# sndels/prosper

Measured on AMD Instinct MI355X. Metric: Mpaths/s, higher is better.
Workload: dtype f32; 1 GPU; S-cornell 1920x1080 8spp maxBounces 4; width=1920, height=1080, spp=8, max_bounces=4, triangles=38, bvh_nodes=7, parallelism=image stripes x1, pipeline=wavefront, 3 frames in flight (one launch chain each)

## Files before the change

include/prosper_pt/prosper_pt.h:

```cpp
#ifndef PROSPER_PT_H
#define PROSPER_PT_H

#include <stddef.h>
#include <stdint.h>

#include "shader_structs.h"

#ifdef __cplusplus
extern "C" {
#endif

#define PROSPER_PT_ABI_VERSION 4

enum
{
    PROSPER_PT_OK = 0,
    PROSPER_PT_ERR_INVALID_ARGUMENT = -1,
    PROSPER_PT_ERR_NO_DEVICE = -2,
    PROSPER_PT_ERR_HIP = -3,
    PROSPER_PT_ERR_NO_SCENE = -4,
    PROSPER_PT_ERR_SCENE = -5,
    PROSPER_PT_ERR_UNSUPPORTED = -6,
    PROSPER_PT_NOT_READY = -7,
};
// ... 969 lines not shown
int prosper_pt_comm_init(prosper_pt_ctx *ctx, const uint8_t id[PROSPER_PT_COMM_ID_BYTES], uint32_t rank, uint32_t ranks);
int prosper_pt_comm_adopt(prosper_pt_ctx *ctx, void *nccl_comm, uint32_t rank, uint32_t ranks);
int prosper_pt_comm_destroy(prosper_pt_ctx *ctx);
int prosper_pt_gather_tiles(
    prosper_pt_ctx *ctx, uint32_t root, void *device_full_rgba32f, size_t byte_size, uint32_t flags, void *stream);
int prosper_pt_gather_wait(prosper_pt_ctx *ctx, void *stream);
typedef struct prosper_pt_comm_info
{
    uint32_t ranks;
    uint32_t rank;
    int32_t device;
    uint32_t gathers;
    float lastGatherMs;
    uint32_t reserved;
} prosper_pt_comm_info;
int prosper_pt_comm_query(prosper_pt_ctx *ctx, prosper_pt_comm_info *out);
int prosper_pt_get_gathered_device_ptr(prosper_pt_ctx *ctx, void **out_ptr, uint32_t *width, uint32_t *height);
int prosper_pt_read_gathered(prosper_pt_ctx *ctx, float *rgba32f, size_t byte_size, void *stream);
int prosper_pt_deinterleave_tiles(
    prosper_pt_ctx *ctx, const void *device_tiles, uint32_t ranks, uint32_t stripe_width, uint32_t width, uint32_t height,
    void *device_full_rgba32f, size_t byte_size, void *stream);

int prosper_pt_get_counters(prosper_pt_ctx *ctx, prosper_pt_counters *out, void *stream);
int prosper_pt_get_stage_counters(prosper_pt_ctx *ctx, uint32_t stage, prosper_pt_counters *out, void *stream);
int prosper_pt_reset_counters(prosper_pt_ctx *ctx, void *stream);

#define PROSPER_PT_MAX_KERNELS 8
int prosper_pt_get_last_render_ms(prosper_pt_ctx *ctx, float *total_ms, float kernel_ms[PROSPER_PT_MAX_KERNELS]);
int prosper_pt_get_last_render_timing(
    prosper_pt_ctx *ctx, float *total_ms, float kernel_ms[PROSPER_PT_MAX_KERNELS],
    uint32_t kernel_launches[PROSPER_PT_MAX_KERNELS]);
const char *prosper_pt_kernel_name(uint32_t index);
int prosper_pt_set_kernel_timing(prosper_pt_ctx *ctx, int enabled);

enum
{
    PROSPER_PT_FN_SINCOS = 0,
    PROSPER_PT_FN_POW = 1,
    PROSPER_PT_FN_SRGB_TO_LINEAR = 2,
    PROSPER_PT_FN_NORMALIZE = 3,
    PROSPER_PT_FN_UNPACK_SNORM = 4,
    PROSPER_PT_FN_ONB = 5,
    PROSPER_PT_FN_COSINE_SAMPLE = 6,
    PROSPER_PT_FN_VNDF_SAMPLE = 7,
    PROSPER_PT_FN_VNDF_PDF = 8,
    PROSPER_PT_FN_EVAL_BRDF = 9,
    PROSPER_PT_FN_OFFSET_RAY = 10,
    PROSPER_PT_FN_POINT_LIGHT = 11,
    PROSPER_PT_FN_SPOT_LIGHT = 12,
    PROSPER_PT_FN_TRIANGLE = 13,
    PROSPER_PT_FN_HALF = 14,
    PROSPER_PT_FN_RNG = 15,
    PROSPER_PT_FN_BC7_BLOCK = 16,
    PROSPER_PT_FN_COUNT = 17,
};

int prosper_pt_debug_srgb_monotonicity(
    prosper_pt_ctx *ctx, uint32_t first_bits, uint32_t last_bits, float *max_defect, uint64_t *decreases);

int prosper_pt_eval_device_fn(
    prosper_pt_ctx *ctx, uint32_t fn, const float *in, uint32_t in_stride, float *out,
    uint32_t out_stride, uint32_t n);

#ifdef __cplusplus
}
#endif

#endif
```

prosper_amd/csrc/prosper_pt.cpp:

```cpp
#include "../../include/prosper_pt/prosper_pt.h"

#include <hip/hip_runtime.h>

#include <algorithm>
#include <chrono>
#include <future>
#include <memory>
#include <cmath>
#include <cstdlib>
#include <cstdio>
#include <cstring>
#include <exception>
#include <stdexcept>
#include <string>
#include <vector>

#include "bvh_build.hpp"
#include "pt_animation.hpp"
#include "pt_context.hpp"
#include "pt_geometry.hpp"
#include "pt_kernels.hpp"
#include "pt_materials.hpp"
#include "pt_pass_support.hpp"
#include "pt_scene.hpp"
// ... 1539 lines not shown
    float total = 0.0f;
    if (const int rc = ctx->timeline.add_to(perStage, launches, &total)) return rc;
    if (perStage[kStageChains] > 0.0f || launches[kStageChains] > 0)
    {
        uint32_t chainLaunches = 0;
        float chainMs = 0.0f;
        for (const LaunchTimeline &chain : ctx->slots[ctx->timedSlot].chains)
        {
            if (const int rc = chain.add_to(perStage, launches, &chainMs)) return rc;
            chainLaunches += chain.intervals();
        }
        if (chainLaunches)
        {
            perStage[kStageChains] = 0.0f;
            launches[kStageChains] = 0;
        }
    }
    *total_ms = total;
    for (int i = 0; i < PROSPER_PT_MAX_KERNELS; ++i)
    {
        if (kernel_ms) kernel_ms[i] = perStage[i];
        if (kernel_launches) kernel_launches[i] = launches[i];
    }
    return PROSPER_PT_OK;
}

int prosper_pt_debug_srgb_monotonicity(
    prosper_pt_ctx *ctx, uint32_t first_bits, uint32_t last_bits, float *max_defect, uint64_t *decreases)
{
    if (!ctx || !max_defect || !decreases || first_bits > last_bits || last_bits >= 0x7F800000u)
        return fail(PROSPER_PT_ERR_INVALID_ARGUMENT, "prosper_pt_debug_srgb_monotonicity: bad argument");
    PPT_HIP(hipSetDevice(ctx->device));
    uint32_t *d = nullptr;
    PPT_HIP(hipMalloc((void **)&d, 8));
    hipError_t e = hipMemset(d, 0, 8);
    uint32_t host[2] = {0u, 0u};
    if (e == hipSuccess)
    {
        launch_srgb_monotonicity(first_bits, last_bits, d, nullptr);
        e = hipGetLastError();
    }
    if (e == hipSuccess) e = hipMemcpy(host, d, 8, hipMemcpyDeviceToHost);
    (void)hipFree(d);
    PPT_HIP(e);
    std::memcpy(max_defect, &host[0], 4);
    *decreases = host[1];
    return PROSPER_PT_OK;
}

int prosper_pt_eval_device_fn(
    prosper_pt_ctx *ctx, uint32_t fn, const float *in, uint32_t in_stride, float *out, uint32_t out_stride, uint32_t n)
{
    if (!ctx || !in || !out || fn >= PROSPER_PT_FN_COUNT || in_stride == 0 || out_stride == 0 ||
        (fn == PROSPER_PT_FN_BC7_BLOCK && (in_stride < 4 || out_stride < 16)))
        return fail(PROSPER_PT_ERR_INVALID_ARGUMENT, "prosper_pt_eval_device_fn: bad argument");
    PPT_HIP(hipSetDevice(ctx->device));
    float *dIn = nullptr, *dOut = nullptr;
    const size_t inBytes = (size_t)n * in_stride * 4, outBytes = (size_t)n * out_stride * 4;
    PPT_HIP(hipMalloc((void **)&dIn, inBytes + 16));
    hipError_t e = hipMalloc((void **)&dOut, outBytes + 16);
    if (e == hipSuccess) e = hipMemcpy(dIn, in, inBytes, hipMemcpyHostToDevice);
    if (e == hipSuccess) e = hipMemset(dOut, 0, outBytes + 16);
    if (e == hipSuccess)
    {
        launch_eval_fn(fn, dIn, in_stride, dOut, out_stride, n, nullptr);
        e = hipGetLastError();
    }
    if (e == hipSuccess) e = hipMemcpy(out, dOut, outBytes, hipMemcpyDeviceToHost);
    (void)hipFree(dIn);
    (void)hipFree(dOut);
    if (e != hipSuccess) return fail(PROSPER_PT_ERR_HIP, std::string("eval_device_fn: ") + hipGetErrorString(e));
    return PROSPER_PT_OK;
}

}
```

prosper_amd/csrc/pt_device.hpp:

```cpp
#pragma once

#include "pt_math.hpp"
#include "pt_scene.hpp"

namespace ppt
{

#define PPT_D __device__ __forceinline__

constexpr uint32_t kMissIndex = 0xFFFFFFFFu;

struct LaneCounters
{
    uint32_t closestRays, shadowRays, nodeVisits, triangleTests, closestHits, anyHitCalls, lightSamples,
        spotLightSamples, skyLookups, shortIndexHits, paths, pixelsWritten, historyReads, shortIndexTriangleTests,
        nodePhaseSteps, trianglePhaseSteps, anyHitTexelFetches;
};


PPT_D uint32_t pcg(uint32_t v)
{
    const uint32_t state = v * 747796405u + 2891336453u;
    const uint32_t word = ((state >> ((state >> 28) + 4u)) ^ state) * 277803737u;
    return (word >> 22) ^ word;
// ... 1452 lines not shown
{
    const float tMaxK = tMax * kSlabTol;
    e[0] = slab_entry(tnx01.x, tny01.x, tnz01.x, tfx01.x, tfy01.x, tfz01.x, tMin, tMaxK);
    e[1] = slab_entry(tnx01.y, tny01.y, tnz01.y, tfx01.y, tfy01.y, tfz01.y, tMin, tMaxK);
    e[2] = slab_entry(tnx23.x, tny23.x, tnz23.x, tfx23.x, tfy23.x, tfz23.x, tMin, tMaxK);
    e[3] = slab_entry(tnx23.y, tny23.y, tnz23.y, tfx23.y, tfy23.y, tfz23.y, tMin, tMaxK);
    ref[0] = (int32_t)children.x;
    ref[1] = (int32_t)children.y;
    ref[2] = (int32_t)children.z;
    ref[3] = (int32_t)children.w;
#define PPT_CSWAP(i, j)                                                                                                \
    {                                                                                                                  \
        const bool sw = e[j] < e[i];                                                                                   \
        const float te = sw ? e[j] : e[i];                                                                             \
        e[j] = sw ? e[i] : e[j];                                                                                       \
        e[i] = te;                                                                                                     \
        const int32_t tr = sw ? ref[j] : ref[i];                                                                       \
        ref[j] = sw ? ref[i] : ref[j];                                                                                 \
        ref[i] = tr;                                                                                                   \
    }
    if constexpr (SORTED)
    {
        PPT_CSWAP(0, 1)
        PPT_CSWAP(2, 3)
        PPT_CSWAP(0, 2)
        PPT_CSWAP(1, 3)
        PPT_CSWAP(1, 2)
    }
#undef PPT_CSWAP
}

template <bool SORTED = true>
PPT_D void intersect_node4(const NodeData &n, f3 o, const RaySlabs &rs, float tMin, float tMax, float e[4], int32_t ref[4])
{
    const float ox = o.x - __builtin_bit_cast(float, n.q0.x);
    const float oy = o.y - __builtin_bit_cast(float, n.q0.y);
    const float oz = o.z - __builtin_bit_cast(float, n.q0.z);
    const bool sx = rs.invd.x < 0.0f, sy = rs.invd.y < 0.0f, sz = rs.invd.z < 0.0f;
    const uint32_t nx01 = sx ? n.q2.z : n.q1.x, nx23 = sx ? n.q2.w : n.q1.y;
    const uint32_t fx01 = sx ? n.q1.x : n.q2.z, fx23 = sx ? n.q1.y : n.q2.w;
    const uint32_t ny01 = sy ? n.q3.x : n.q1.z, ny23 = sy ? n.q3.y : n.q1.w;
    const uint32_t fy01 = sy ? n.q1.z : n.q3.x, fy23 = sy ? n.q1.w : n.q3.y;
    const uint32_t nz01 = sz ? n.q3.z : n.q2.x, nz23 = sz ? n.q3.w : n.q2.y;
    const uint32_t fz01 = sz ? n.q2.x : n.q3.z, fz23 = sz ? n.q2.y : n.q3.w;
    const v2f tnx01 = plane_offsets(nx01, ox) * rs.invd.x, tnx23 = plane_offsets(nx23, ox) * rs.invd.x;
    const v2f tny01 = plane_offsets(ny01, oy) * rs.invd.y, tny23 = plane_offsets(ny23, oy) * rs.invd.y;
    const v2f tnz01 = plane_offsets(nz01, oz) * rs.invd.z, tnz23 = plane_offsets(nz23, oz) * rs.invd.z;
    const v2f tfx01 = plane_offsets(fx01, ox) * rs.invdK.x, tfx23 = plane_offsets(fx23, ox) * rs.invdK.x;
    const v2f tfy01 = plane_offsets(fy01, oy) * rs.invdK.y, tfy23 = plane_offsets(fy23, oy) * rs.invdK.y;
    const v2f tfz01 = plane_offsets(fz01, oz) * rs.invdK.z, tfz23 = plane_offsets(fz23, oz) * rs.invdK.z;
    finish_node4<SORTED>(tnx01, tnx23, tny01, tny23, tnz01, tnz23, tfx01, tfx23, tfy01, tfy23, tfz01, tfz23, n.q4, tMin, tMax, e, ref);
}

struct GlobalGeom
{
    const BvhNode *nodes;
    const WorldTriangle *triangles;
    PPT_D NodeData node(int32_t i) const
    {
        const uint4 *np = reinterpret_cast<const uint4 *>(nodes + i);
        return NodeData{np[0], np[1], np[2], np[3], np[4]};
    }
    template <bool SORTED>
    PPT_D void test_node(int32_t i, f3 o, const RaySlabs &rs, float tMin, float tMax, float e[4], int32_t ref[4]) const
    {
        intersect_node4<SORTED>(node(i), o, rs, tMin, tMax, e, ref);
    }
    PPT_D TriangleData tri(uint32_t i) const
    {
        const float4 *tp = reinterpret_cast<const float4 *>(triangles + i);
        return TriangleData{tp[0], tp[1], tp[2]};
    }
};
constexpr uint32_t kLdsNodeStride = 9;
struct LdsGeom
{
    const float4 *nodes;
    const float4 *triangles;
    template <bool SORTED>
    PPT_D void test_node(int32_t i, f3 o, const RaySlabs &rs, float tMin, float tMax, float e[4], int32_t ref[4]) const
    {
        typedef float f4n __attribute__((ext_vector_type(4)));
        typedef uint32_t u4n __attribute__((ext_vector_type(4)));
        typedef __attribute__((address_space(3))) const f4n *lds_f4;
        typedef __attribute__((address_space(3))) const u4n *lds_u4;
        const uint32_t base = (uint32_t)(uintptr_t)(__attribute__((address_space(3))) const void *)nodes + (uint32_t)i * (kLdsNodeStride * 16u);
        const uint32_t sx = (__builtin_bit_cast(uint32_t, rs.invd.x) >> 25) & 64u;
        const uint32_t sy = (__builtin_bit_cast(uint32_t, rs.invd.y) >> 25) & 64u;
        const uint32_t sz = (__builtin_bit_cast(uint32_t, rs.invd.z) >> 25) & 64u;
        const f4n origin = *(lds_f4)(uintptr_t)(base);
        const f4n nx = *(lds_f4)(uintptr_t)(base + 16u + sx), fx = *(lds_f4)(uintptr_t)(base + 80u - sx);
        const f4n ny = *(lds_f4)(uintptr_t)(base + 32u + sy), fy = *(lds_f4)(uintptr_t)(base + 96u - sy);
        const f4n nz = *(lds_f4)(uintptr_t)(base + 48u + sz), fz = *(lds_f4)(uintptr_t)(base + 112u - sz);
        const u4n ch = *(lds_u4)(uintptr_t)(base + 64u);
        const uint4 children = make_uint4(ch.x, ch.y, ch.z, ch.w);
        const float ox = o.x - origin.x, oy = o.y - origin.y, oz = o.z - origin.z;
        const v2f tnx01 = v2f{nx.x - ox, nx.y - ox} * rs.invd.x, tnx23 = v2f{nx.z - ox, nx.w - ox} * rs.invd.x;
        const v2f tny01 = v2f{ny.x - oy, ny.y - oy} * rs.invd.y, tny23 = v2f{ny.z - oy, ny.w - oy} * rs.invd.y;
        const v2f tnz01 = v2f{nz.x - oz, nz.y - oz} * rs.invd.z, tnz23 = v2f{nz.z - oz, nz.w - oz} * rs.invd.z;
        const v2f tfx01 = v2f{fx.x - ox, fx.y - ox} * rs.invdK.x, tfx23 = v2f{fx.z - ox, fx.w - ox} * rs.invdK.x;
        const v2f tfy01 = v2f{fy.x - oy, fy.y - oy} * rs.invdK.y, tfy23 = v2f{fy.z - oy, fy.w - oy} * rs.invdK.y;
        const v2f tfz01 = v2f{fz.x - oz, fz.y - oz} * rs.invdK.z, tfz23 = v2f{fz.z - oz, fz.w - oz} * rs.invdK.z;
        finish_node4<SORTED>(tnx01, tnx23, tny01, tny23, tnz01, tnz23, tfx01, tfx23, tfy01, tfy23, tfz01, tfz23, children, tMin, tMax, e, ref);
    }
    PPT_D TriangleData tri(uint32_t i) const
    {
        const float4 *tp = triangles + i * 3u;
        return TriangleData{tp[0], tp[1], tp[2]};
    }
};
constexpr uint32_t kLdsNodeStrideHalf = 5;
struct LdsGeomHalf
{
    const float4 *nodes;
    const float4 *triangles;
    PPT_D NodeData node(int32_t i) const
    {
        const uint4 *np = reinterpret_cast<const uint4 *>(nodes + (uint32_t)i * kLdsNodeStrideHalf);
        return NodeData{np[0], np[1], np[2], np[3], np[4]};
    }
    template <bool SORTED>
    PPT_D void test_node(int32_t i, f3 o, const RaySlabs &rs, float tMin, float tMax, float e[4], int32_t ref[4]) const
    {
        intersect_node4<SORTED>(node(i), o, rs, tMin, tMax, e, ref);
    }
    PPT_D TriangleData tri(uint32_t i) const
    {
        const float4 *tp = triangles + i * 3u;
        return TriangleData{tp[0], tp[1], tp[2]};
    }
};
constexpr uint32_t kLdsSceneFloat4s = 768;

PPT_D bool descend_any(const float e[4], const int32_t ref[4], const TraversalStack &stack, int32_t &sp, int32_t &node)
{
    bool found = false;
    if (stack.ldsOnly || (uint32_t)sp + 3u <= stack.cap)
    {
#pragma unroll
        for (int k = 0; k < 4; ++k)
            if (e[k] < kInf)
            {
                if (found)
                    stack.lds[(uint32_t)(sp++) * stack.ldsStride] = ref[k];
                else
                {
                    node = ref[k];
                    found = true;
                }
            }
        return found;
    }
#pragma unroll
    for (int k = 0; k < 4; ++k)
        if (e[k] < kInf)
        {
            if (found)
                stack.push(sp, ref[k]);
            else
            {
                node = ref[k];
                found = true;
            }
        }
    return found;
}

enum BlendPolicy : uint32_t
{
    kBlendStochastic = 0,
    kBlendReject = 1,
    kBlendPeel = 2,
};
PPT_D bool ascending(f3 a, f3 b)
{
    return a.x < b.x || (a.x == b.x && (a.y < b.y || (a.y == b.y && a.z < b.z)));
}

template <bool ANY, bool COUNT, class Geom, BlendPolicy BLEND = kBlendStochastic>
PPT_D bool trace_in(
    const Geom &g, const DeviceScene &s, f3 o, f3 d, float tMin, float tMaxIn, uint32_t seed, const TraversalStack &stack,
    Hit &hit, LaneCounters &cnt, const Hit *after = nullptr)
// ... 309 lines not shown
```

prosper_amd/csrc/pt_kernels.hip:

```cpp
#include "pt_kernels.hpp"

#include "bvh_encode.hpp"
#include "pt_bc7.hpp"
#include "pt_device.hpp"
#include "pt_render_common.hpp"

namespace ppt
{


__global__ void flatten_triangles_kernel(
    DeviceScene s, const uint32_t *__restrict__ triOffsets, uint32_t drawInstanceCount,
    const uint32_t *__restrict__ drawInstanceFlags, WorldTriangle *__restrict__ out,
    ShadeTriangle *__restrict__ shadeOut, AlphaTriangle *__restrict__ alphaOut, uint32_t total,
    const uint32_t *__restrict__ leafPosition, WorldTriangle *__restrict__ leafOrder)
{
    const uint32_t g = blockIdx.x * blockDim.x + threadIdx.x;
    if (g >= total) return;
    uint32_t lo = 0, hi = drawInstanceCount;
    while (hi - lo > 1)
    {
        const uint32_t mid = (lo + hi) >> 1;
        if (triOffsets[mid] <= g)
            lo = mid;
// ... 557 lines not shown
        break;
    case PROSPER_PT_FN_EVAL_BRDF:
    {
        Surface sf = {};
        sf.normalWS = f3{a[3], a[4], a[5]};
        sf.invViewRayWS = f3{a[6], a[7], a[8]};
        sf.material.albedo = f3{a[9], a[10], a[11]};
        sf.material.roughness = a[12];
        sf.material.metallic = a[13];
        sf.NoV = saturate(dot(sf.normalWS, sf.invViewRayWS));
        const f3 r = eval_brdf_times_nol(f3{a[0], a[1], a[2]}, sf);
        o[0] = r.x; o[1] = r.y; o[2] = r.z;
        break;
    }
    case PROSPER_PT_FN_OFFSET_RAY:
    {
        const f3 r = offset_ray(f3{a[0], a[1], a[2]}, f3{a[3], a[4], a[5]});
        o[0] = r.x; o[1] = r.y; o[2] = r.z;
        break;
    }
    case PROSPER_PT_FN_POINT_LIGHT:
    {
        prosper_PointLight L;
        L.position = prosper_vec4{a[0], a[1], a[2], 0.0f};
        L.radianceAndRadius = prosper_vec4{a[3], a[4], a[5], a[6]};
        f3 l, irr;
        float d;
        eval_point_light(L, f3{a[7], a[8], a[9]}, l, d, irr);
        o[0] = l.x; o[1] = l.y; o[2] = l.z; o[3] = d; o[4] = irr.x; o[5] = irr.y; o[6] = irr.z;
        break;
    }
    case PROSPER_PT_FN_SPOT_LIGHT:
    {
        prosper_SpotLight L;
        L.positionAndAngleOffset = prosper_vec4{a[0], a[1], a[2], a[3]};
        L.radianceAndAngleScale = prosper_vec4{a[4], a[5], a[6], a[7]};
        L.direction = prosper_vec4{a[8], a[9], a[10], 0.0f};
        f3 l, irr;
        float d;
        eval_spot_light(L, f3{a[11], a[12], a[13]}, l, d, irr);
        o[0] = l.x; o[1] = l.y; o[2] = l.z; o[3] = d; o[4] = irr.x; o[5] = irr.y; o[6] = irr.z;
        break;
    }
    case PROSPER_PT_FN_TRIANGLE:
    {
        float t = 0.0f, bu = 0.0f, bv = 0.0f;
        const f3 dir = f3{a[3], a[4], a[5]};
        const bool hit = intersect_triangle(
            f3{a[0], a[1], a[2]}, dir, f3{safe_rcp_dir(dir.x), safe_rcp_dir(dir.y), safe_rcp_dir(dir.z)},
            f3{a[6], a[7], a[8]}, f3{a[9], a[10], a[11]}, f3{a[12], a[13], a[14]}, a[15], a[16], t, bu, bv);
        o[0] = hit ? 1.0f : 0.0f; o[1] = hit ? t : 0.0f; o[2] = hit ? bu : 0.0f; o[3] = hit ? bv : 0.0f;
        break;
    }
    case PROSPER_PT_FN_HALF:
    {
        const uint32_t h = float_to_half(a[0]);
        o[0] = half_to_float(h);
        o[1] = u2f(h);
        break;
    }
    case PROSPER_PT_FN_RNG:
    {
        Rng r{f2u(a[0]), f2u(a[1]), f2u(a[2])};
        o[0] = r.rnd01();
        const f2 u = r.rnd2d01();
        o[1] = u.x; o[2] = u.y;
        o[3] = u2f(pcg(r.x ^ r.z));
        break;
    }
    case PROSPER_PT_FN_BC7_BLOCK:
    {
        const uint32_t block[4] = {f2u(a[0]), f2u(a[1]), f2u(a[2]), f2u(a[3])};
        uint32_t texel[16];
        bc7_decode_block(block, texel);
        for (int k = 0; k < 16; ++k) o[k] = u2f(texel[k]);
        break;
    }
    default: break;
    }
}

__global__ __launch_bounds__(256) void decode_bc7_kernel(
    const uint4 *__restrict__ blocks, uint32_t blocksX, uint32_t blocksY, uint32_t tilesPerRow, uint32_t *__restrict__ tiled)
{
    const uint32_t i = blockIdx.x * blockDim.x + threadIdx.x;
    if (i >= blocksX * blocksY) return;
    const uint4 raw = blocks[i];
    const uint32_t block[4] = {raw.x, raw.y, raw.z, raw.w};
    uint32_t texel[16];
    bc7_decode_block(block, texel);
    const uint32_t bx = i % blocksX, by = i / blocksX;
    uint32_t *tile = tiled + ((size_t)by * tilesPerRow + (bx >> 1)) * (kTexTileW * kTexTileH) + (bx & 1u) * 4u;
    for (uint32_t row = 0; row < 4u; ++row)
        *reinterpret_cast<uint4 *>(tile + row * kTexTileW) =
            make_uint4(texel[row * 4u], texel[row * 4u + 1u], texel[row * 4u + 2u], texel[row * 4u + 3u]);
}

void launch_decode_bc7(
    const void *blocks, uint32_t width, uint32_t height, uint32_t tilesPerRow, void *tiled, hipStream_t stream)
{
    const uint32_t blocksX = width / 4u, blocksY = height / 4u;
    const uint32_t n = blocksX * blocksY;
    if (n == 0) return;
    hipLaunchKernelGGL(
        decode_bc7_kernel, dim3((n + 255u) / 256u), dim3(256), 0, stream, static_cast<const uint4 *>(blocks), blocksX, blocksY,
        tilesPerRow, static_cast<uint32_t *>(tiled));
// ... 180 lines not shown
```

prosper_amd/csrc/pt_trace_stream.hpp:

```cpp
#pragma once

#include "pt_device.hpp"

#ifndef PPT_TRI_BEATS_NODE
#define PPT_TRI_BEATS_NODE(t, n) (2u * (t) > 3u * (n))
#endif
#ifndef PPT_REFILL
#define PPT_REFILL(r, best) ((r) >= 32u)
#endif
#ifndef PPT_CONTINUE
#define PPT_CONTINUE(c, c0, other) (3u * (c) > (c0))
#endif
#ifndef PPT_ANY_BEATS
#define PPT_ANY_BEATS(a, best) (4u * (a) > (best))
#endif

namespace ppt
{

PPT_D f3 xyz3(float4 v) { return f3{v.x, v.y, v.z}; }

enum : uint32_t
{
    kLaneIdle = 0,
    kLaneNode = 1,
    kLaneTri = 2,
    kLaneAny = 3,
    kLaneFinished = 4,
};

struct StreamRay
{
    f3 o, d;
    float tMin, tMax;
    uint32_t seed;
};

template <bool ANY, bool COUNT, class Geom, class Fetch, class Commit>
PPT_D void trace_stream(
    const Geom &g, const DeviceScene &s, uint32_t n, const TraversalStack &stack, LaneCounters &cnt, Fetch &&fetch,
    Commit &&commit)
{
    const uint32_t lane = threadIdx.x & 63u;
    const unsigned long long below = (1ull << lane) - 1ull;

    uint32_t next = 0;
    uint32_t state = kLaneIdle;
    uint32_t ray = 0;
    f3 o = {}, d = {}, invd = {};
    RaySlabs rs = {};
    float tMin = 0.0f, tMaxIn = 0.0f;
    uint32_t seed = 0;
    int32_t node = 0, sp = 0;
    uint32_t triFirst = 0, triCount = 0;
    Hit hit = {};
    uint32_t cAlpha = 0;
    float cT = 0.0f, cBu = 0.0f, cBv = 0.0f;

    auto pop = [&]() {
        if (sp == 0)
            state = kLaneFinished;
        else
        {
            node = stack.pop(sp);
            if (node >= 0)
                state = kLaneNode;
            else
            {
                const uint32_t ref = (uint32_t)~node;
                triFirst = ref >> 3;
                triCount = (ref & 7u) + 1u;
                state = kLaneTri;
            }
// ... 38 lines not shown
            const uint32_t other = nTri > nAny ? (nTri > nRefill ? nTri : nRefill) : (nAny > nRefill ? nAny : nRefill);
            (void)other;
            uint32_t c = nNode;
            do
            {
                if constexpr (COUNT) cnt.nodePhaseSteps += lane == 0 ? 1u : 0u;
                if (state == kLaneNode)
                {
                    if constexpr (COUNT) cnt.nodeVisits++;
                    float e[4];
                    int32_t ref[4];
                    bool entered;
                    if constexpr (ANY)
                    {
                        g.template test_node<false>(node, o, rs, tMin, hit.t, e, ref);
                        entered = descend_any(e, ref, stack, sp, node);
                    }
                    else
                    {
                        g.template test_node<true>(node, o, rs, tMin, hit.t, e, ref);
                        stack.push_hit_children(sp, e, ref);
                        entered = e[0] < kInf;
                        if (entered) node = ref[0];
                    }
                    if (entered)
                    {
                        if (node < 0)
                        {
                            const uint32_t leaf = (uint32_t)~node;
                            triFirst = leaf >> 3;
                            triCount = (leaf & 7u) + 1u;
                            state = kLaneTri;
                        }
                    }
                    else
                        pop();
                }
                c = (uint32_t)__builtin_popcountll(__ballot(state == kLaneNode));
            } while (PPT_CONTINUE(c, nNode, other));
        }
        else if (pick == kLaneTri)
        {
            const uint32_t other = nNode > nAny ? (nNode > nRefill ? nNode : nRefill) : (nAny > nRefill ? nAny : nRefill);
            (void)other;
            uint32_t c = nTri;
            do
            {
                if constexpr (COUNT) cnt.trianglePhaseSteps += lane == 0 ? 1u : 0u;
                const bool inTri = state == kLaneTri;
                const bool two = inTri && triCount >= 2u;
                const bool anyTwo = __any(two);
                if (inTri)
                {
                    TriangleData td = g.tri(triFirst);
                    EdgeFunctions e = edge_functions(o, d, xyz3(td.a), xyz3(td.b), xyz3(td.c));
                    uint32_t consumed = 1u;
                    if (anyTwo)
                    {
                        const TriangleData td2 = g.tri(two ? triFirst + 1u : triFirst);
                        EdgeFunctions e2 = edge_functions(o, d, xyz3(td2.a), xyz3(td2.b), xyz3(td2.c));
                        e2.pass = e2.pass && two;
                        if (two && !(e.pass && e2.pass)) consumed = 2u;
                        if (!e.pass && e2.pass)
                        {
                            td = td2;
                            e = e2;
                        }
                    }
                    const float4 a = td.a, b = td.b, c4 = td.c;
                    triFirst += consumed;
                    triCount -= consumed;
                    if constexpr (COUNT)
                    {
                        cnt.triangleTests += consumed;
                        cnt.shortIndexTriangleTests +=
                            (__builtin_bit_cast(uint32_t, c4.w) & kTriFlagShortIndices) ? consumed : 0u;
                    }
                    float t, bu, bv;
                    bool candidate =
                        e.pass && finish_triangle(e, o, d, invd, xyz3(a), xyz3(b), xyz3(c4), tMin, tMaxIn, t, bu, bv);
                    const uint32_t di = __builtin_bit_cast(uint32_t, a.w);
                    const uint32_t prim = __builtin_bit_cast(uint32_t, b.w);
                    const uint32_t flags = __builtin_bit_cast(uint32_t, c4.w);
                    if (candidate && !ANY && hit.drawInstance != kMissIndex)
                    {
                        if (t > hit.t) candidate = false;
                        if (t == hit.t && !(di < hit.drawInstance || (di == hit.drawInstance && prim < hit.primitive)))
                            candidate = false;
                    }
                    if (candidate)
                    {
                        if (flags & kTriFlagOpaque)
                            accept(di, prim, t, bu, bv);
                        else
                        {
                            cAlpha = flags >> kTriAlphaShift;
                            cT = t;
                            cBu = bu;
                            cBv = bv;
                            state = kLaneAny;
                        }
                    }
                    if (state == kLaneTri && triCount == 0) pop();
                }
                c = (uint32_t)__builtin_popcountll(__ballot(state == kLaneTri));
            } while (PPT_CONTINUE(c, nTri, other));
        }
        else if (pick == kLaneAny)
        {
            if (state == kLaneAny)
            {
                state = kLaneTri;
                if (any_hit_record<COUNT>(s, cAlpha, f2{cBu, cBv}, seed, cnt))
                {
                    const AlphaTriangle *rec = s.alphaTriangles + cAlpha;
                    accept(rec->drawInstance, rec->primitive, cT, cBu, cBv);
                }
                if (state == kLaneTri && triCount == 0) pop();
            }
        }
        else
        {
            commit(state == kLaneFinished, ray, hit.drawInstance != kMissIndex, hit, d);
            if (state == kLaneFinished) state = kLaneIdle;
            const unsigned long long mIdle = __ballot(state == kLaneIdle);
            const uint32_t rank = (uint32_t)__builtin_popcountll(mIdle & below);
            const uint32_t idx = next + rank;
            if (state == kLaneIdle && idx < n)
            {
                ray = idx;
                const StreamRay r = fetch(idx);
                o = r.o;
                d = r.d;
                tMin = r.tMin;
                tMaxIn = r.tMax;
                seed = r.seed;
                invd = f3{safe_rcp_dir(d.x), safe_rcp_dir(d.y), safe_rcp_dir(d.z)};
                rs = make_ray_slabs(invd);
                hit.drawInstance = kMissIndex;
                hit.primitive = kMissIndex;
                hit.bary = f2{0.0f, 0.0f};
                hit.t = tMaxIn;
                sp = 0;
                node = 0;
                state = kLaneNode;
            }
            const uint32_t handed = (uint32_t)__builtin_popcountll(mIdle);
            next = (n - next < handed) ? n : next + handed;
        }
    }
}

}
```

prosper_amd/csrc/pt_wavefront.hip:

```cpp
#include "pt_kernels.hpp"

#include "pt_device.hpp"
#include "pt_render_common.hpp"
#include "pt_trace_stream.hpp"

#define PPT_SHADE_WPE 4
#ifndef PPT_GEN_WPE
#define PPT_GEN_WPE 5
#endif
#ifndef PPT_TRACE_WPE
#define PPT_TRACE_WPE(stack) 5
#endif

namespace ppt
{

namespace
{

constexpr uint32_t kSlotMask = 0x0FFFFFFFu;

struct SegmentId
{
    uint32_t seg;
// ... 174 lines not shown
    r.py = ty * 8u + iy;
    r.slot = r.frame * w.pixelsPadded + tile * 64u + iy * 8u + ix;
    r.valid = inRange && rank < tiles && r.frame < frames && r.lx < p.localWidth && r.py < p.height;
    return r;
}

__device__ __forceinline__ void add_to_slot(float4 *color, uint32_t slot, uint32_t flags, f3 value, uint32_t bounce)
{
#if PPT_STREAM_NT & 4
    const ppt_f4v cv = __builtin_nontemporal_load(reinterpret_cast<const ppt_f4v *>(color + slot));
    float4 c = make_float4(cv.x, cv.y, cv.z, cv.w);
#else
    float4 c = color[slot];
#endif
    f3 acc = f3{c.x, c.y, c.z};
    add_bounce(flags, acc, value, bounce);
#if PPT_STREAM_NT & 4
    __builtin_nontemporal_store(ppt_f4v{acc.x, acc.y, acc.z, 0.0f}, reinterpret_cast<ppt_f4v *>(color + slot));
#else
    color[slot] = make_float4(acc.x, acc.y, acc.z, 0.0f);
#endif
}

__device__ __forceinline__ LdsGeomHalf stage_scene_in_lds_half(const DeviceScene &s, float4 *lds, uint32_t nodeCount, uint32_t triCount)
{
    const float4 *gn = reinterpret_cast<const float4 *>(s.nodes);
    for (uint32_t i = threadIdx.x; i < nodeCount * kLdsNodeStrideHalf; i += blockDim.x) lds[i] = gn[i];
    float4 *lt = lds + nodeCount * kLdsNodeStrideHalf;
    const float4 *gt = reinterpret_cast<const float4 *>(s.triangles);
    for (uint32_t i = threadIdx.x; i < triCount * 3u; i += blockDim.x) lt[i] = gt[i];
    __syncthreads();
    return LdsGeomHalf{lds, lt};
}

__device__ __forceinline__ LdsGeom stage_scene_in_lds(const DeviceScene &s, float4 *lds, uint32_t nodeCount, uint32_t triCount)
{
    const BvhNode *gn = s.nodes;
    float *lf = reinterpret_cast<float *>(lds);
    for (uint32_t i = threadIdx.x; i < nodeCount * (kLdsNodeStride * 4u); i += blockDim.x)
    {
        const uint32_t n = i / (kLdsNodeStride * 4u), k = i - n * (kLdsNodeStride * 4u);
        const uint32_t q = k >> 2, c = k & 3u;
        float v = 0.0f;
        if (q == 0u)
            v = c < 3u ? gn[n].origin[c] : 0.0f;
        else if (q >= 1u && q <= 3u)
            v = half_to_float(gn[n].lo[q - 1u][c]);
        else if (q == 4u)
            v = __builtin_bit_cast(float, gn[n].child[c]);
        else if (q <= 7u)
            v = half_to_float(gn[n].hi[q - 5u][c]);
        lf[i] = v;
    }
    float4 *lt = lds + nodeCount * kLdsNodeStride;
    const float4 *gt = reinterpret_cast<const float4 *>(s.triangles);
    for (uint32_t i = threadIdx.x; i < triCount * 3u; i += blockDim.x) lt[i] = gt[i];
    __syncthreads();
    return LdsGeom{lds, lt};
}

}


template <bool COUNT, int STACK, bool LDS_SCENE>
__global__ __launch_bounds__(256, PPT_GEN_WPE) void wf_generate_extend(
    DeviceScene s, RenderParams p, WavefrontBuffers w, uint32_t nodeCount, uint32_t triCount,
    int32_t *__restrict__ stackOverflow, unsigned long long *__restrict__ counters)
{
    __shared__ int32_t ldsStack[STACK * 256];
    __shared__ float4 ldsScene[LDS_SCENE ? kLdsSceneFloat4s : 1];
    LdsGeomHalf lg = {};
    if constexpr (LDS_SCENE) lg = stage_scene_in_lds_half(s, ldsScene, nodeCount, triCount);
    const GlobalGeom gg{s.nodes, s.triangles};
    const SegmentId id = my_segment(w);
    if (!id.valid) return;
    const uint32_t lane = lane_id();
    const TraversalStack stack{(lds_int32 *)ldsStack + (threadIdx.x >> 6) * (STACK * 64u) + lane,
                               stackOverflow + blockIdx.x * 256u + threadIdx.x, (uint32_t)STACK, gridDim.x * 256u, 64u, LDS_SCENE};
    const bool traceRays = p.pc.maxBounces > 0;

    LaneCounters cnt = {};
    uint32_t nHit = 0;
    if (!traceRays)
    {
        for (uint32_t k = lane; k < w.segLen; k += 64u)
        {
            const SlotPixel sp = decode_slot(w, p, id.base + k);
            if (sp.valid)
            {
                if constexpr (COUNT) cnt.paths++;
                w.color[id.base + k] = make_float4(0.0f, 0.0f, 0.0f, 0.0f);
            }
        }
    }
    else
    {
        BatchLane bl = {};
        auto fetch = [&](uint32_t k) {
            const uint32_t at = id.base + k;
            StreamRay r;
            if (!bl.valid)
            {
                r.o = f3{0.0f, 0.0f, 0.0f};
                r.d = f3{0.0f, 0.0f, 1.0f};
                r.tMin = 0.0f;
                r.tMax = -1.0f;
                r.seed = 0;
                return r;
            }
            PathState st;
            start_path<COUNT>(p, local_to_global_x(p, bl.lx), bl.py, (p.pc.frameIndex + bl.frame) % PROSPER_RT_FRAME_PERIOD,
// ... 386 lines not shown
                       *cTrace = counters + kStageTrace * kCounterCount;
    auto mark = [&](uint32_t st) {
        if (timer) timer->mark(st, stream);
    };
    const dim3 grid(((w.groupCount + 7u) / 8u) * 8u), block(256);
    uint32_t bounces = p.pc.maxBounces < PROSPER_RT_MAX_BOUNCES ? p.pc.maxBounces : PROSPER_RT_MAX_BOUNCES;
    const bool debugDraw =
        p.pc.drawType != PROSPER_DRAW_TYPE_DEFAULT && p.pc.drawType != PROSPER_DRAW_TYPE_MESHLET_ID;
    if (debugDraw && bounces > 1) bounces = 1;

    mark(kStageGenerate);
    hipLaunchKernelGGL(
        (wf_generate_extend<COUNT, STACK, LDS_SCENE>), grid, block, 0, stream, s, p, w, nodeCount, triCount,
        stackOverflow, cGen);
    for (uint32_t b = 0; b < bounces; ++b)
    {
        const uint32_t cur = b & 1u;
        const uint32_t last = (b + 1u == bounces) ? 1u : 0u;
        mark(kStageShade);
        const int ldsTables = !plan.tablesInLds ? 0 : (shade_table_bytes(s, true) <= kLdsTableBytes ? 1 : 2);
        auto shade = [&](auto kernel) { hipLaunchKernelGGL(kernel, grid, block, 0, stream, s, p, w, b, cur, last, cShade); };
        if (s.batchedTextures)
            ldsTables == 1 ? shade(wf_shade<COUNT, 1, true>) : (ldsTables == 2 ? shade(wf_shade<COUNT, 2, true>) : shade(wf_shade<COUNT, 0, true>));
        else
            ldsTables == 1 ? shade(wf_shade<COUNT, 1, false>) : (ldsTables == 2 ? shade(wf_shade<COUNT, 2, false>) : shade(wf_shade<COUNT, 0, false>));
        if (!debugDraw)
        {
            mark(kStageTrace);
            hipLaunchKernelGGL(
                (wf_trace<COUNT, STACK, LDS_SCENE>), grid, block, 0, stream, s, p, w, b, cur ^ 1u, last ? 0u : 1u,
                nodeCount, triCount, stackOverflow, cTrace);
        }
    }
}

uint32_t wavefront_grid_blocks(const WavefrontBuffers &w)
{
    const uint32_t groups = (w.nSeg + 3u) / 4u;
    return ((groups + 7u) / 8u) * 8u + 8u * kMaxChains;
}

uint32_t wavefront_lds_stack_entries(uint32_t stackBound, uint32_t forced)
{
    if (forced == 16u || forced == 24u || forced == 32u) return forced;
    return stackBound <= 16u ? 16u : 24u;
}

bool wavefront_shade_tables_in_lds(const DeviceScene &s, bool disabled)
{
    return shade_table_bytes(s, false) <= kLdsTableBytes && !disabled;
}
bool wavefront_scene_in_lds(uint32_t ldsStackEntries, uint32_t stackBound, uint32_t nodeCount, uint32_t triCount, bool disabled)
{
    return ldsStackEntries == 16u && stackBound <= 16u && nodeCount * kLdsNodeStride + triCount * 3u <= kLdsSceneFloat4s && !disabled;
}

WavefrontPlan wavefront_plan(
    uint32_t stackBound, uint32_t nodeCount, uint32_t triCount, const DeviceScene &s, const WavefrontOptions &opt)
{
    WavefrontPlan plan = {};
    plan.ldsStackEntries = wavefront_lds_stack_entries(stackBound, opt.ldsStackEntries);
    plan.overflowEntries = stackBound > plan.ldsStackEntries ? stackBound - plan.ldsStackEntries : 0u;
    plan.sceneInLds = wavefront_scene_in_lds(plan.ldsStackEntries, stackBound, nodeCount, triCount, opt.noLdsScene);
    plan.tablesInLds = wavefront_shade_tables_in_lds(s, opt.noLdsTables);
    plan.scratchDwordsPerBlock = plan.overflowEntries * 256u;
    return plan;
}

template <bool COUNT>
static void enqueue_for_stack(
    const DeviceScene &s, const RenderParams &p, unsigned long long *counters, const WavefrontBuffers &w,
    const WavefrontPlan &plan, int32_t *stackOverflow, uint32_t nodeCount, uint32_t triCount, LaunchTimeline *timer,
    hipStream_t stream)
{
    if (plan.sceneInLds)
        enqueue_wavefront<COUNT, 16, true>(s, p, counters, w, plan, nodeCount, triCount, stackOverflow, timer, stream);
    else if (plan.ldsStackEntries == 16u)
        enqueue_wavefront<COUNT, 16, false>(s, p, counters, w, plan, nodeCount, triCount, stackOverflow, timer, stream);
    else if (plan.ldsStackEntries == 24u)
        enqueue_wavefront<COUNT, 24, false>(s, p, counters, w, plan, nodeCount, triCount, stackOverflow, timer, stream);
    else
        enqueue_wavefront<COUNT, 32, false>(s, p, counters, w, plan, nodeCount, triCount, stackOverflow, timer, stream);
}

void launch_render_wavefront(
    const DeviceScene &s, const RenderParams &p, float4 *hdr, unsigned long long *counters, const WavefrontBuffers &w,
    const WavefrontPlan &plan, int32_t *stackOverflow, uint32_t nodeCount, uint32_t triCount, bool countWork,
    LaunchTimeline *timer, const WavefrontChains &chains, hipStream_t stream)
{
    if (w.nSeg == 0) return;
    static_assert(kTraversalStackDepth == 32, "largest LDS stack variant");
    const uint32_t groups = (w.nSeg + 3u) / 4u;
    uint32_t parts = chains.count < kMaxChains ? chains.count : kMaxChains;
    while (parts > 1u && groups < 256u * parts) --parts;
    const bool ownStreams = parts > 1u || chains.detached;
    const uint32_t per = (groups + parts - 1u) / parts;
    const bool forked = parts > 1u && !chains.detached;
    if (forked) (void)chains.fork->record(stream);
    uint32_t blocksBefore = 0;
    for (uint32_t i = 0; i < parts; ++i)
    {
        WavefrontBuffers part = w;
        part.groupBase = i * per;
        part.groupCount = (part.groupBase + per <= groups) ? per : groups - part.groupBase;
        hipStream_t cs = ownStreams ? chains.streams[i] : stream;
        LaunchTimeline *ct = ownStreams ? chains.timers[i] : timer;
        if (forked) (void)chains.fork->wait(cs);
// ... 28 lines not shown
```

Before: 8831 Mpaths/s.

## Transpose LDS triangles to SoA and test triangle pairs with precomputed guard boxes

Stores LDS-resident triangles in a structure-of-arrays layout so adjacent triangles load as two-wide vectors, and evaluates both triangles' edge functions together. The old guard check, which recomputed vertex distances in finish_triangle, is replaced by a padded bounding box per triangle that is precomputed in LDS during staging. Other parts: mbcnt replaces the popcount used for lane rank, the far-plane slab scale is recomputed per node with asm barriers that stop values being hoisted into extra registers, and new eval_device_fn test hooks are added. This adds LDS footprint and changes the LDS-fit criterion, and the guard semantics could differ slightly at the tolerance edges.

```diff
diff --git a/include/prosper_pt/prosper_pt.h b/include/prosper_pt/prosper_pt.h
--- a/include/prosper_pt/prosper_pt.h
+++ b/include/prosper_pt/prosper_pt.h
@@ -1045,7 +1045,9 @@
     PROSPER_PT_FN_HALF = 14,
     PROSPER_PT_FN_RNG = 15,
     PROSPER_PT_FN_BC7_BLOCK = 16,
-    PROSPER_PT_FN_COUNT = 17,
+    PROSPER_PT_FN_TRIANGLE_PAIR = 17,
+    PROSPER_PT_FN_GUARD_BOX = 18,
+    PROSPER_PT_FN_COUNT = 19,
 };
 
 int prosper_pt_debug_srgb_monotonicity(
diff --git a/prosper_amd/csrc/prosper_pt.cpp b/prosper_amd/csrc/prosper_pt.cpp
--- a/prosper_amd/csrc/prosper_pt.cpp
+++ b/prosper_amd/csrc/prosper_pt.cpp
@@ -1615,7 +1615,9 @@
     prosper_pt_ctx *ctx, uint32_t fn, const float *in, uint32_t in_stride, float *out, uint32_t out_stride, uint32_t n)
 {
     if (!ctx || !in || !out || fn >= PROSPER_PT_FN_COUNT || in_stride == 0 || out_stride == 0 ||
-        (fn == PROSPER_PT_FN_BC7_BLOCK && (in_stride < 4 || out_stride < 16)))
+        (fn == PROSPER_PT_FN_BC7_BLOCK && (in_stride < 4 || out_stride < 16)) ||
+        (fn == PROSPER_PT_FN_TRIANGLE_PAIR && (in_stride < 26 || out_stride < 8)) ||
+        (fn == PROSPER_PT_FN_GUARD_BOX && (in_stride < 9 || out_stride < 6)))
         return fail(PROSPER_PT_ERR_INVALID_ARGUMENT, "prosper_pt_eval_device_fn: bad argument");
     PPT_HIP(hipSetDevice(ctx->device));
     float *dIn = nullptr, *dOut = nullptr;
diff --git a/prosper_amd/csrc/pt_device.hpp b/prosper_amd/csrc/pt_device.hpp
--- a/prosper_amd/csrc/pt_device.hpp
+++ b/prosper_amd/csrc/pt_device.hpp
@@ -1528,8 +1528,127 @@
     finish_node4<SORTED>(tnx01, tnx23, tny01, tny23, tnz01, tnz23, tfx01, tfx23, tfy01, tfy23, tfz01, tfz23, n.q4, tMin, tMax, e, ref);
 }
 
+PPT_D f3 xyz3(float4 v) { return f3{v.x, v.y, v.z}; }
+
+template <bool COUNT, class Geom>
+PPT_D bool triangle_step_scalar(
+    const Geom &g, uint32_t &triFirst, uint32_t &triCount, bool two, bool anyTwo, f3 o, f3 d, f3 invd, float tMin, float tMax,
+    LaneCounters &cnt, float &t, float &bu, float &bv, uint32_t &drawInstance, uint32_t &primitive, uint32_t &flags)
+{
+    TriangleData td = g.tri(triFirst);
+    EdgeFunctions e = edge_functions(o, d, xyz3(td.a), xyz3(td.b), xyz3(td.c));
+    uint32_t consumed = 1u;
+    if (anyTwo)
+    {
+        const TriangleData td2 = g.tri(two ? triFirst + 1u : triFirst);
+        EdgeFunctions e2 = edge_functions(o, d, xyz3(td2.a), xyz3(td2.b), xyz3(td2.c));
+        e2.pass = e2.pass && two;
+        if (two && !(e.pass && e2.pass)) consumed = 2u;
+        if (!e.pass && e2.pass)
+        {
+            td = td2;
+            e = e2;
+        }
+    }
+    const float4 a = td.a, b = td.b, c4 = td.c;
+    triFirst += consumed;
+    triCount -= consumed;
+    if constexpr (COUNT)
+    {
+        cnt.triangleTests += consumed;
+        cnt.shortIndexTriangleTests += (__builtin_bit_cast(uint32_t, c4.w) & kTriFlagShortIndices) ? consumed : 0u;
+    }
+    const bool candidate = e.pass && finish_triangle(e, o, d, invd, xyz3(a), xyz3(b), xyz3(c4), tMin, tMax, t, bu, bv);
+    drawInstance = __builtin_bit_cast(uint32_t, a.w);
+    primitive = __builtin_bit_cast(uint32_t, b.w);
+    flags = __builtin_bit_cast(uint32_t, c4.w);
+    return candidate;
+}
+
+PPT_D void per_step(float &x) { asm volatile("" : "+v"(x)); }
+PPT_D void per_step(f3 &v) { per_step(v.x), per_step(v.y), per_step(v.z); }
+struct EdgeFunctionsPair
+{
+    v2f ax, ay, az, bx, by, bz, cx, cy, cz;
+    v2f U, V, W, det;
+};
+struct EdgeOperands
+{
+    f3 A, B, C;
+    float U, V, W, det;
+};
+PPT_D bool edge_functions_pass(float U, float V, float W, float det)
+{
+    const bool mixed = (U < 0.0f || V < 0.0f || W < 0.0f) && (U > 0.0f || V > 0.0f || W > 0.0f);
+    return !mixed && det != 0.0f;
+}
+PPT_D EdgeFunctionsPair edge_functions_pair(f3 o, f3 d, v2f v0x, v2f v0y, v2f v0z, v2f v1x, v2f v1y, v2f v1z, v2f v2x, v2f v2y, v2f v2z)
+{
+    EdgeFunctionsPair e;
+    for (int h = 0; h < 2; ++h)
+    {
+        const f3 A = f3{v0x[h], v0y[h], v0z[h]} - o, B = f3{v1x[h], v1y[h], v1z[h]} - o, C = f3{v2x[h], v2y[h], v2z[h]} - o;
+        e.ax[h] = A.x, e.ay[h] = A.y, e.az[h] = A.z, e.bx[h] = B.x, e.by[h] = B.y, e.bz[h] = B.z, e.cx[h] = C.x, e.cy[h] = C.y, e.cz[h] = C.z;
+        e.U[h] = dot(d, cross(C, B));
+        e.V[h] = dot(d, cross(A, C));
+        e.W[h] = dot(d, cross(B, A));
+        e.det[h] = (e.U[h] + e.V[h]) + e.W[h];
+    }
+    return e;
+}
+PPT_D EdgeOperands edge_operands(const EdgeFunctionsPair &e, bool second)
+{
+    EdgeOperands r;
+    r.A = second ? f3{e.ax.y, e.ay.y, e.az.y} : f3{e.ax.x, e.ay.x, e.az.x};
+    r.B = second ? f3{e.bx.y, e.by.y, e.bz.y} : f3{e.bx.x, e.by.x, e.bz.x};
+    r.C = second ? f3{e.cx.y, e.cy.y, e.cz.y} : f3{e.cx.x, e.cy.x, e.cz.x};
+    r.U = second ? e.U.y : e.U.x;
+    r.V = second ? e.V.y : e.V.x;
+    r.W = second ? e.W.y : e.W.x;
+    r.det = second ? e.det.y : e.det.x;
+    return r;
+}
+
+struct GuardBox
+{
+    v2f x, y, z;
+};
+PPT_D GuardBox guard_box(f3 v0, f3 v1, f3 v2)
+{
+    const float lox = fminf(fminf(v0.x, v1.x), v2.x), hix = fmaxf(fmaxf(v0.x, v1.x), v2.x);
+    const float loy = fminf(fminf(v0.y, v1.y), v2.y), hiy = fmaxf(fmaxf(v0.y, v1.y), v2.y);
+    const float loz = fminf(fminf(v0.z, v1.z), v2.z), hiz = fmaxf(fmaxf(v0.z, v1.z), v2.z);
+    const float mx = fmaxf(fabs_(lox), fabs_(hix));
+    const float my = fmaxf(fabs_(loy), fabs_(hiy));
+    const float mz = fmaxf(fabs_(loz), fabs_(hiz));
+    const float pad = fmaxf(fmaxf(mx, my), mz) * kGuardPad;
+    return GuardBox{v2f{lox - pad, hix + pad}, v2f{loy - pad, hiy + pad}, v2f{loz - pad, hiz + pad}};
+}
+PPT_D bool box_guard(f3 o, f3 invd, const GuardBox &g, float tt)
+{
+    const v2f x = (g.x - o.x) * invd.x;
+    const v2f y = (g.y - o.y) * invd.y;
+    const v2f z = (g.z - o.z) * invd.z;
+    const float tn = fmaxf(fmaxf(fminf(x.x, x.y), fminf(y.x, y.y)), fminf(z.x, z.y));
+    const float tf = fminf(fminf(fmaxf(x.x, x.y), fmaxf(y.x, y.y)), fmaxf(z.x, z.y));
+    return tn <= tt * kGuardTol && tt <= tf * kGuardTol;
+}
+PPT_D bool finish_triangle(
+    const EdgeOperands &e, f3 o, f3 d, f3 invd, const GuardBox &g, float tMin, float tMax, float &t, float &bu, float &bv)
+{
+    const float inv = 1.0f / e.det;
+    const float tt = __builtin_fmaf(e.W, dot(e.C, d), __builtin_fmaf(e.V, dot(e.B, d), e.U * dot(e.A, d))) * inv;
+    if (!(tt > tMin && tt < tMax)) return false;
+    if (!box_guard(o, invd, g, tt)) return false;
+    t = tt;
+    bu = e.V * inv;
+    bv = e.W * inv;
+    return true;
+}
+
 struct GlobalGeom
 {
+    static constexpr bool kLeanRegisters = false;
     const BvhNode *nodes;
     const WorldTriangle *triangles;
     PPT_D NodeData node(int32_t i) const
@@ -1547,20 +1666,38 @@
         const float4 *tp = reinterpret_cast<const float4 *>(triangles + i);
         return TriangleData{tp[0], tp[1], tp[2]};
     }
+    template <bool COUNT>
+    PPT_D bool triangle_step(
+        uint32_t &triFirst, uint32_t &triCount, bool two, bool anyTwo, f3 o, f3 d, f3 invd, float tMin, float tMax, LaneCounters &cnt,
+        float &t, float &bu, float &bv, uint32_t &drawInstance, uint32_t &primitive, uint32_t &flags) const
+    {
+        return triangle_step_scalar<COUNT>(
+            *this, triFirst, triCount, two, anyTwo, o, d, invd, tMin, tMax, cnt, t, bu, bv, drawInstance, primitive, flags);
+    }
 };
 constexpr uint32_t kLdsNodeStride = 9;
+constexpr uint32_t kLdsTriStride = 84;
+constexpr uint32_t kLdsTriMax = kLdsTriStride - 1u;
+constexpr uint32_t kLdsTriFloat4s = 12u * kLdsTriStride / 4u;
+constexpr uint32_t lds_scene_float4s(uint32_t nodeCount, uint32_t triCount)
+{
+    return nodeCount * kLdsNodeStride + kLdsTriFloat4s + (triCount * 6u + 3u) / 4u;
+}
 struct LdsGeom
 {
+    static constexpr bool kLeanRegisters = true;
     const float4 *nodes;
-    const float4 *triangles;
+    const float *triangles;
+    const v2f *guards;
     template <bool SORTED>
-    PPT_D void test_node(int32_t i, f3 o, const RaySlabs &rs, float tMin, float tMax, float e[4], int32_t ref[4]) const
+    PPT_D void test_node(int32_t i, f3 o, RaySlabs &rs, float tMin, float tMax, float e[4], int32_t ref[4]) const
     {
         typedef float f4n __attribute__((ext_vector_type(4)));
         typedef uint32_t u4n __attribute__((ext_vector_type(4)));
         typedef __attribute__((address_space(3))) const f4n *lds_f4;
         typedef __attribute__((address_space(3))) const u4n *lds_u4;
         const uint32_t base = (uint32_t)(uintptr_t)(__attribute__((address_space(3))) const void *)nodes + (uint32_t)i * (kLdsNodeStride * 16u);
+        per_step(rs.invd);
         const uint32_t sx = (__builtin_bit_cast(uint32_t, rs.invd.x) >> 25) & 64u;
         const uint32_t sy = (__builtin_bit_cast(uint32_t, rs.invd.y) >> 25) & 64u;
         const uint32_t sz = (__builtin_bit_cast(uint32_t, rs.invd.z) >> 25) & 64u;
@@ -1574,20 +1711,55 @@
         const v2f tnx01 = v2f{nx.x - ox, nx.y - ox} * rs.invd.x, tnx23 = v2f{nx.z - ox, nx.w - ox} * rs.invd.x;
         const v2f tny01 = v2f{ny.x - oy, ny.y - oy} * rs.invd.y, tny23 = v2f{ny.z - oy, ny.w - oy} * rs.invd.y;
         const v2f tnz01 = v2f{nz.x - oz, nz.y - oz} * rs.invd.z, tnz23 = v2f{nz.z - oz, nz.w - oz} * rs.invd.z;
-        const v2f tfx01 = v2f{fx.x - ox, fx.y - ox} * rs.invdK.x, tfx23 = v2f{fx.z - ox, fx.w - ox} * rs.invdK.x;
-        const v2f tfy01 = v2f{fy.x - oy, fy.y - oy} * rs.invdK.y, tfy23 = v2f{fy.z - oy, fy.w - oy} * rs.invdK.y;
-        const v2f tfz01 = v2f{fz.x - oz, fz.y - oz} * rs.invdK.z, tfz23 = v2f{fz.z - oz, fz.w - oz} * rs.invdK.z;
+        const float kx = rs.invd.x * kSlabTol, ky = rs.invd.y * kSlabTol, kz = rs.invd.z * kSlabTol;
+        const v2f tfx01 = v2f{fx.x - ox, fx.y - ox} * kx, tfx23 = v2f{fx.z - ox, fx.w - ox} * kx;
+        const v2f tfy01 = v2f{fy.x - oy, fy.y - oy} * ky, tfy23 = v2f{fy.z - oy, fy.w - oy} * ky;
+        const v2f tfz01 = v2f{fz.x - oz, fz.y - oz} * kz, tfz23 = v2f{fz.z - oz, fz.w - oz} * kz;
         finish_node4<SORTED>(tnx01, tnx23, tny01, tny23, tnz01, tnz23, tfx01, tfx23, tfy01, tfy23, tfz01, tfz23, children, tMin, tMax, e, ref);
     }
-    PPT_D TriangleData tri(uint32_t i) const
-    {
-        const float4 *tp = triangles + i * 3u;
-        return TriangleData{tp[0], tp[1], tp[2]};
+    template <bool COUNT>
+    PPT_D bool triangle_step(
+        uint32_t &triFirst, uint32_t &triCount, bool two, bool, f3 &o, f3 &d, f3 &invd, float tMin, float tMax, LaneCounters &cnt,
+        float &t, float &bu, float &bv, uint32_t &drawInstance, uint32_t &primitive, uint32_t &flags) const
+    {
+        typedef v2f v2fu __attribute__((aligned(4)));
+        typedef __attribute__((address_space(3))) const v2fu *lds_v2f;
+        typedef __attribute__((address_space(3))) const v2f *lds_v2f8;
+        constexpr uint32_t kArray = kLdsTriStride * 4u;
+        per_step(o), per_step(d), per_step(invd);
+        const uint32_t base = (uint32_t)(uintptr_t)(__attribute__((address_space(3))) const void *)triangles + triFirst * 4u;
+        auto comp = [&](uint32_t k) { return *(lds_v2f)(uintptr_t)(base + k * kArray); };
+        typedef uint32_t v2u __attribute__((ext_vector_type(2)));
+        typedef v2u v2uu __attribute__((aligned(4)));
+        typedef __attribute__((address_space(3))) const v2uu *lds_v2u;
+        const EdgeFunctionsPair e = edge_functions_pair(o, d, comp(0), comp(1), comp(2), comp(4), comp(5), comp(6), comp(8), comp(9), comp(10));
+        const v2u words[3] = {*(lds_v2u)(uintptr_t)(base + 3u * kArray), *(lds_v2u)(uintptr_t)(base + 7u * kArray), *(lds_v2u)(uintptr_t)(base + 11u * kArray)};
+        const bool pass0 = edge_functions_pass(e.U.x, e.V.x, e.W.x, e.det.x);
+        const bool pass1 = edge_functions_pass(e.U.y, e.V.y, e.W.y, e.det.y) && two;
+        const uint32_t consumed = (two && !(pass0 && pass1)) ? 2u : 1u;
+        const bool second = !pass0 && pass1;
+        const uint32_t chosen = triFirst + (second ? 1u : 0u);
+        auto word = [&](uint32_t k) { return second ? words[k >> 2].y : words[k >> 2].x; };
+        triFirst += consumed;
+        triCount -= consumed;
+        if constexpr (COUNT)
+        {
+            cnt.triangleTests += consumed;
+            cnt.shortIndexTriangleTests += (word(11) & kTriFlagShortIndices) ? consumed : 0u;
+        }
+        if (!(pass0 || pass1)) return false;
+        const uint32_t gb = (uint32_t)(uintptr_t)(__attribute__((address_space(3))) const void *)guards + chosen * 24u;
+        const GuardBox g{*(lds_v2f8)(uintptr_t)(gb), *(lds_v2f8)(uintptr_t)(gb + 8u), *(lds_v2f8)(uintptr_t)(gb + 16u)};
+        drawInstance = word(3);
+        primitive = word(7);
+        flags = word(11);
+        return finish_triangle(edge_operands(e, second), o, d, invd, g, tMin, tMax, t, bu, bv);
     }
 };
 constexpr uint32_t kLdsNodeStrideHalf = 5;
 struct LdsGeomHalf
 {
+    static constexpr bool kLeanRegisters = false;
     const float4 *nodes;
     const float4 *triangles;
     PPT_D NodeData node(int32_t i) const
@@ -1604,6 +1776,14 @@
     {
         const float4 *tp = triangles + i * 3u;
         return TriangleData{tp[0], tp[1], tp[2]};
+    }
+    template <bool COUNT>
+    PPT_D bool triangle_step(
+        uint32_t &triFirst, uint32_t &triCount, bool two, bool anyTwo, f3 o, f3 d, f3 invd, float tMin, float tMax, LaneCounters &cnt,
+        float &t, float &bu, float &bv, uint32_t &drawInstance, uint32_t &primitive, uint32_t &flags) const
+    {
+        return triangle_step_scalar<COUNT>(
+            *this, triFirst, triCount, two, anyTwo, o, d, invd, tMin, tMax, cnt, t, bu, bv, drawInstance, primitive, flags);
     }
 };
 constexpr uint32_t kLdsSceneFloat4s = 768;
diff --git a/prosper_amd/csrc/pt_kernels.hip b/prosper_amd/csrc/pt_kernels.hip
--- a/prosper_amd/csrc/pt_kernels.hip
+++ b/prosper_amd/csrc/pt_kernels.hip
@@ -633,6 +633,32 @@
         o[0] = hit ? 1.0f : 0.0f; o[1] = hit ? t : 0.0f; o[2] = hit ? bu : 0.0f; o[3] = hit ? bv : 0.0f;
         break;
     }
+    case PROSPER_PT_FN_TRIANGLE_PAIR:
+    {
+        const f3 org = f3{a[0], a[1], a[2]}, dir = f3{a[3], a[4], a[5]};
+        const f3 invd = f3{safe_rcp_dir(dir.x), safe_rcp_dir(dir.y), safe_rcp_dir(dir.z)};
+        const float *p = a + 6, *q = a + 15;
+        const EdgeFunctionsPair e = edge_functions_pair(
+            org, dir, v2f{p[0], q[0]}, v2f{p[1], q[1]}, v2f{p[2], q[2]}, v2f{p[3], q[3]}, v2f{p[4], q[4]}, v2f{p[5], q[5]},
+            v2f{p[6], q[6]}, v2f{p[7], q[7]}, v2f{p[8], q[8]});
+        for (int h = 0; h < 2; ++h)
+        {
+            const float *v = h ? q : p;
+            const EdgeOperands eo = edge_operands(e, h != 0);
+            const GuardBox g = guard_box(f3{v[0], v[1], v[2]}, f3{v[3], v[4], v[5]}, f3{v[6], v[7], v[8]});
+            float t = 0.0f, bu = 0.0f, bv = 0.0f;
+            const bool hit = edge_functions_pass(eo.U, eo.V, eo.W, eo.det) &&
+                             finish_triangle(eo, org, dir, invd, g, a[24], a[25], t, bu, bv);
+            o[4 * h] = hit ? 1.0f : 0.0f; o[4 * h + 1] = hit ? t : 0.0f; o[4 * h + 2] = hit ? bu : 0.0f; o[4 * h + 3] = hit ? bv : 0.0f;
+        }
+        break;
+    }
+    case PROSPER_PT_FN_GUARD_BOX:
+    {
+        const GuardBox g = guard_box(f3{a[0], a[1], a[2]}, f3{a[3], a[4], a[5]}, f3{a[6], a[7], a[8]});
+        o[0] = g.x.x; o[1] = g.x.y; o[2] = g.y.x; o[3] = g.y.y; o[4] = g.z.x; o[5] = g.z.y;
+        break;
+    }
     case PROSPER_PT_FN_HALF:
     {
         const uint32_t h = float_to_half(a[0]);
diff --git a/prosper_amd/csrc/pt_trace_stream.hpp b/prosper_amd/csrc/pt_trace_stream.hpp
--- a/prosper_amd/csrc/pt_trace_stream.hpp
+++ b/prosper_amd/csrc/pt_trace_stream.hpp
@@ -17,8 +17,6 @@
 
 namespace ppt
 {
-
-PPT_D f3 xyz3(float4 v) { return f3{v.x, v.y, v.z}; }
 
 enum : uint32_t
 {
@@ -163,36 +161,10 @@
                 const bool anyTwo = __any(two);
                 if (inTri)
                 {
-                    TriangleData td = g.tri(triFirst);
-                    EdgeFunctions e = edge_functions(o, d, xyz3(td.a), xyz3(td.b), xyz3(td.c));
-                    uint32_t consumed = 1u;
-                    if (anyTwo)
-                    {
-                        const TriangleData td2 = g.tri(two ? triFirst + 1u : triFirst);
-                        EdgeFunctions e2 = edge_functions(o, d, xyz3(td2.a), xyz3(td2.b), xyz3(td2.c));
-                        e2.pass = e2.pass && two;
-                        if (two && !(e.pass && e2.pass)) consumed = 2u;
-                        if (!e.pass && e2.pass)
-                        {
-                            td = td2;
-                            e = e2;
-                        }
-                    }
-                    const float4 a = td.a, b = td.b, c4 = td.c;
-                    triFirst += consumed;
-                    triCount -= consumed;
-                    if constexpr (COUNT)
-                    {
-                        cnt.triangleTests += consumed;
-                        cnt.shortIndexTriangleTests +=
-                            (__builtin_bit_cast(uint32_t, c4.w) & kTriFlagShortIndices) ? consumed : 0u;
-                    }
                     float t, bu, bv;
-                    bool candidate =
-                        e.pass && finish_triangle(e, o, d, invd, xyz3(a), xyz3(b), xyz3(c4), tMin, tMaxIn, t, bu, bv);
-                    const uint32_t di = __builtin_bit_cast(uint32_t, a.w);
-                    const uint32_t prim = __builtin_bit_cast(uint32_t, b.w);
-                    const uint32_t flags = __builtin_bit_cast(uint32_t, c4.w);
+                    uint32_t di, prim, flags;
+                    bool candidate = g.template triangle_step<COUNT>(
+                        triFirst, triCount, two, anyTwo, o, d, invd, tMin, tMaxIn, cnt, t, bu, bv, di, prim, flags);
                     if (candidate && !ANY && hit.drawInstance != kMissIndex)
                     {
                         if (t > hit.t) candidate = false;
@@ -235,7 +207,11 @@
             commit(state == kLaneFinished, ray, hit.drawInstance != kMissIndex, hit, d);
             if (state == kLaneFinished) state = kLaneIdle;
             const unsigned long long mIdle = __ballot(state == kLaneIdle);
-            const uint32_t rank = (uint32_t)__builtin_popcountll(mIdle & below);
+            uint32_t rank;
+            if constexpr (Geom::kLeanRegisters)
+                rank = __builtin_amdgcn_mbcnt_hi((uint32_t)(mIdle >> 32), __builtin_amdgcn_mbcnt_lo((uint32_t)mIdle, 0u));
+            else
+                rank = (uint32_t)__builtin_popcountll(mIdle & below);
             const uint32_t idx = next + rank;
             if (state == kLaneIdle && idx < n)
             {
diff --git a/prosper_amd/csrc/pt_wavefront.hip b/prosper_amd/csrc/pt_wavefront.hip
--- a/prosper_amd/csrc/pt_wavefront.hip
+++ b/prosper_amd/csrc/pt_wavefront.hip
@@ -250,11 +250,27 @@
             v = half_to_float(gn[n].hi[q - 5u][c]);
         lf[i] = v;
     }
-    float4 *lt = lds + nodeCount * kLdsNodeStride;
+    float *lt = lf + nodeCount * (kLdsNodeStride * 4u);
+    v2f *lg = reinterpret_cast<v2f *>(lt + kLdsTriFloat4s * 4u);
     const float4 *gt = reinterpret_cast<const float4 *>(s.triangles);
-    for (uint32_t i = threadIdx.x; i < triCount * 3u; i += blockDim.x) lt[i] = gt[i];
+    for (uint32_t i = threadIdx.x; i <= triCount; i += blockDim.x)
+    {
+        const float4 zero = make_float4(0.0f, 0.0f, 0.0f, 0.0f);
+        const bool real = i < triCount;
+        const float4 a = real ? gt[i * 3u] : zero, b = real ? gt[i * 3u + 1u] : zero, c = real ? gt[i * 3u + 2u] : zero;
+        const float v[12] = {a.x, a.y, a.z, a.w, b.x, b.y, b.z, b.w, c.x, c.y, c.z, c.w};
+#pragma unroll
+        for (uint32_t k = 0; k < 12u; ++k) lt[k * kLdsTriStride + i] = v[k];
+        if (real)
+        {
+            const GuardBox g = guard_box(xyz3(a), xyz3(b), xyz3(c));
+            lg[i * 3u] = g.x;
+            lg[i * 3u + 1u] = g.y;
+            lg[i * 3u + 2u] = g.z;
+        }
+    }
     __syncthreads();
-    return LdsGeom{lds, lt};
+    return LdsGeom{lds, lt, lg};
 }
 
 }
@@ -747,7 +763,9 @@
 }
 bool wavefront_scene_in_lds(uint32_t ldsStackEntries, uint32_t stackBound, uint32_t nodeCount, uint32_t triCount, bool disabled)
 {
-    return ldsStackEntries == 16u && stackBound <= 16u && nodeCount * kLdsNodeStride + triCount * 3u <= kLdsSceneFloat4s && !disabled;
+    const bool fits = triCount <= kLdsTriMax && nodeCount * kLdsNodeStrideHalf + triCount * 3u <= kLdsSceneFloat4s &&
+                      lds_scene_float4s(nodeCount, triCount) <= kLdsSceneFloat4s;
+    return ldsStackEntries == 16u && stackBound <= 16u && fits && !disabled;
 }
 
 WavefrontPlan wavefront_plan(
```

Result: no change. 8843 Mpaths/s, median of 2 (+0.1%).
